# QuackenbushLab/phoenix

Measured on AMD Instinct MI355X. Metric: ODE-RHS evals/sec (genes x trajectories), higher is better.
Workload: dtype f32; 1 GPU; C4 breast_cancer ~11k-gene pseudotime, 256 trajectory intervals/GPU, dopri5 + adjoint; genes=11165, hidden=40, trajectories_per_gpu=256, method=dopri5, parallelism=trajectory-sharded x1, grouped gradient all-reduce, status_readback=deferred

## Files before the change

### phoenix_amd/csrc/phx_adj3.hip

```cpp
#include <hip/hip_runtime.h>

#include <algorithm>
#include <cstdint>
#include <cstdlib>
#include <cstring>

#include "phx_solver.hpp"
#include "phx_host.hpp"

using namespace phxh;

#include "phx_mfma_common.inc"
#include "phx_mfma_v3common.inc"
#include "phx_mfma_adj3.inc"

namespace {

int adj3_mode()
{
    if (force_v0()) return -1;
    const char *e = getenv("PHX_ADJ");
    if (!e) return 0;
    if (strcmp(e, "v3") == 0) return 1;
    if (strcmp(e, "v1") == 0 || strcmp(e, "v2") == 0) return -1;
    return 0;
}

bool plan_adj3(int N, int H, int B, int T, int control, int method, D1 *out)
{
    const int cus = num_cus();
    const int mode = adj3_mode();
    if (cus <= 0 || mode < 0 || method != PHX_DOPRI5 || H > 48) return false;
    const int HT = 3;
    const size_t blkbytes = (size_t)blk_floats_ch(HT, H) * 4;
    const int nblk = (N + 31) / 32, ntt = (B + 15) / 16;
    long long best_cost = -1;
    D1 best{};
    for (int NW = 4; NW >= 1; NW >>= 1)
        for (int TPW = 1; TPW <= 4; TPW <<= 1) {
            const int slots = NW * TPW, TG = (ntt + slots - 1) / slots;
            const int ntg = TG == 1 ? std::min(slots, ntt) : slots, Bt = 16 * ntg;
            const bool helpers = ntg < slots;
            if (control == PHX_CTRL_SHARED && TG != 1) continue;
            const size_t cb = ((ctl3_bytes(Bt, ntg) + 15) & ~(size_t)15) +
                              (v3_split_parts(TG, NW, TPW, ntg) > 1 ? v3_comb_bytes(NW, 4 * HT) : 0);
            if (cb + blkbytes > LDS_BUDGET) continue;
            const int NBmax = (int)std::min<size_t>((LDS_BUDGET - cb) / blkbytes, 8);
            const char *enb = getenv("PHX_V3_NB");
            for (int NB = enb ? std::max(1, atoi(enb)) : 1; NB <= NBmax; ++NB) {
                const int G = (nblk + NB - 1) / NB;
                if ((long long)TG * G > cus) continue;
                const long long cost = (long long)TPW * NB * 1000 + Bt / 4 - (helpers && TPW == 1 ? 50 : 0);
                if (best_cost < 0 || cost < best_cost) {
                    best_cost = cost;
                    best.N = N; best.H = H; best.B = B; best.T = T; best.HT = HT; best.NB = NB; best.NW = NW;
                    best.TPW = TPW; best.G = G; best.TG = TG; best.nblk = nblk; best.ntg = ntg; best.Bt = Bt;
                    best.nvec = NVEC_ADJ3; best.BN = (long long)B * N; best.HC = 1; best.Hc = H;
                    best.Bcall = 0; best.cntN = (long long)B * N;
                }
                break;
            }
        }
    if (best_cost < 0) return false;
    if (mode == 0 && best.G <= 32) return false;
    *out = best;
    return true;
}

size_t pp_adj3(const D1 &d) { return align_up((size_t)d.nblk * (4 * d.HT * 2 * 256) + d.N + 2 * d.H, 64); }


Regions make_layout3(const D1 &d, bool grads)
{
    Regions L{};
    Take take;
    const size_t R = (size_t)d.ntg * 4 * d.HT * 4 + d.ntg;
    L.cnt = take(4096);
    L.part = take((size_t)d.TG * d.G * R * 64 * 8);
    L.zbuf = take((size_t)d.TG * R * 64 * 8);
    L.xbytes = take.off - L.part;
    L.part1 = take((size_t)d.TG * d.G * R * 64 * 8);
    L.zbuf1 = take((size_t)d.TG * R * 64 * 8);
    L.scratch = take((size_t)d.TG * d.G * NVEC_ADJ3 * d.ntg * d.NB * 512 * 4);
    L.pp = (long long)pp_adj3(d);
    L.nparts = d.TG;
    L.dtheta = take(grads ? pp_adj3(d) * 4 * d.TG : 0);
    L.prof = take((size_t)d.TG * d.G * 16 * 8);
    L.wimg = take((size_t)d.nblk * blk_floats_ch(d.HT, d.H) * 4);
    L.hq = take(grads ? (size_t)d.TG * d.ntg * 7 * 4 * d.HT * 1024 : 0);
    L.total = take.off;
    return L;
}

size_t lds_bytes_adj3(const D1 &d)
{
    return (size_t)blk_floats_ch(d.HT, d.H) * 4 * d.NB + ((ctl3_bytes(d.Bt, d.ntg) + 15) & ~(size_t)15) +
           (v3_split_parts(d.TG, d.NW, d.TPW, d.ntg) > 1 ? v3_comb_bytes(d.NW, 4 * d.HT) : 0);
}

const void *prepare_adj3(SolveArgs &a, const phx_params *p, hipStream_t st)
{
    const D1 &d = a.d;
    if (p->wimg) a.w.wimg = (const float *)p->wimg;
    else
        hipLaunchKernelGGL(k1_pack_images, dim3(d.nblk), dim3(256), 0, st, to_net(p), (float *)a.w.wimg, d.HT, 1, p->H,
                           blk_floats_ch(d.HT, p->H));
    a.lds = lds_bytes_adj3(d);
    const char *eh = getenv("PHX_V3_HALF");
    const bool half = p->H <= 16 * (d.HT - 1) + 8 && !(eh && eh[0] == '0');
    const bool split = v3_split_parts(d.TG, d.NW, d.TPW, d.ntg) > 1;
    return split ? (half ? reinterpret_cast<const void *>(k1_solve_adj3<3, true, true>)
                         : reinterpret_cast<const void *>(k1_solve_adj3<3, false, true>))
                 : (half ? reinterpret_cast<const void *>(k1_solve_adj3<3, true, false>)
                         : reinterpret_cast<const void *>(k1_solve_adj3<3, false, false>));
}

hipError_t launch_adj3(const void *fn, const SolveArgs &a, hipStream_t st)
{
    const int flags = a.grads | (a.w.prof_level == 2 ? 2 : 0) | (a.w.prof_level == 3 ? 4 : 0);
    return launch_persistent(fn, dim3(a.d.TG * a.d.G), dim3(64 * a.d.NW), a.lds, st, a.net, a.d, a.w, a.cfg, a.t, a.y_saved,
                             a.grad_y, a.adj_y0, a.status, a.nfe, a.nsteps, flags, a.PP);
}

bool reduce_adj3(const SolveArgs &a, int npart, const phx_grads *g, int overwrite, hipStream_t st)
{
    const D1 &d = a.d;
    const long long total = (long long)d.nblk * (4 * d.HT * 2 * 64) + d.N + 2 * d.H;
    hipLaunchKernelGGL((k3_reduce_grads<3>), dim3((unsigned int)((total + 255) / 256)), dim3(256), 0, st, a.w.dtheta, npart,
                       a.PP, d.N, d.H, d.nblk, g->Ws, g->Wp, g->WaT, g->g, g->bs, g->bp, overwrite, g->Wa);
    return hipGetLastError() == hipSuccess;
}

}

namespace phxh {
const Backend &adj3_backend()
{
    static const Backend b = {3, true, false, true, plan_adj3, make_layout3, plan6_ht, prepare_adj3, launch_adj3, reduce_adj3};
    return b;
}
}
```

### phoenix_amd/csrc/phx_engine.hip

```cpp
#include <hip/hip_runtime.h>

#include <algorithm>
#include <atomic>
#include <cstdint>
#include <cstdio>
#include <cstring>
#include <cstdlib>

#include "phx_solver.hpp"
#include "phx_host.hpp"

using namespace phxh;

namespace {


struct Dims {
    int N, H, B, T;
    int NC;
    int items;
    int GB;
    int BG;
    int Bc;
    long long BN;
// ... 861 lines not shown
                     : reinterpret_cast<const void *>(k1_solve_adj<8, 256, false>);
}

hipError_t launch_v1_fwd(const void *fn, const SolveArgs &a, hipStream_t st)
{
    return launch_plain(fn, dim3(a.d.TG * a.d.G), dim3(64 * a.d.NW), a.lds, st, a.net, a.d, a.w, a.cfg, a.y0, a.t, a.sol,
                        a.status, a.nfe, a.nsteps);
}

hipError_t launch_v1_adj(const void *fn, const SolveArgs &a, hipStream_t st)
{
    return launch_plain(fn, dim3(a.d.TG * a.d.G), dim3(64 * a.d.NW), a.lds, st, a.net, a.d, a.w, a.cfg, a.t, a.y_saved,
                        a.grad_y, a.adj_y0, a.status, a.nfe, a.nsteps, a.grads, a.PP);
}

bool reduce_v1(const SolveArgs &a, int npart, const phx_grads *g, int overwrite, hipStream_t st)
{
    return launch_reduce_grads(a.w.dtheta, npart, a.PP, a.d.N, a.d.H, g, overwrite, st);
}

const Backend &v1_fwd_backend()
{
    static const Backend b = {1, false, false, false,
                                    plan_v1_fwd, layout_v1_fwd, plan6_ht, prepare_v1_fwd, launch_v1_fwd, nullptr, true};
    return b;
}
const Backend &v1_adj_backend()
{
    static const Backend b = {1, false, false, false,
                                    plan_v1_adj, layout_v1_adj, plan6_ht, prepare_v1_adj, launch_v1_adj, reduce_v1, true};
    return b;
}

const Backend *const *backends(int op)
{
    static const Backend *const fwd[] = {&fwd3_backend(), &fwd3c_backend(), &v1_fwd_backend(), nullptr};
    static const Backend *const adj[] = {&adj3_backend(), &adj3c_backend(), &adj2_backend(), &v1_adj_backend(), nullptr};
    static const Backend *const none[] = {nullptr};
    return op == PHX_OP_ODEINT ? fwd : op == PHX_OP_ADJOINT ? adj : none;
}

int pick_chunk(const Backend &be, int N, int H, int B, int T, int control, int method)
{
    D1 d;
    if (be.plan(N, H, B, T, control, method, &d)) return B;
    if (control != PHX_CTRL_PER_TRAJECTORY) return 0;
    for (int bc = 4096; bc >= 16; bc >>= 1)
        if (bc < B && be.plan(N, H, bc, T, control, method, &d)) return bc;
    return 0;
}

struct Pick {
    const Backend *be;
    int chunk;
};

Pick first_backend(int op, int N, int H, int B, int T, int control, int method, bool whole = false, bool stepped = false)
{
    for (const Backend *const *b = backends(op); *b; ++b) {
        D1 d;
        if (stepped && !(*b)->substeps) continue;
        const int chunk = !whole ? pick_chunk(**b, N, H, B, T, control, method)
                                 : (*b)->plan(N, H, B, T, control, method, &d) ? B : 0;
        if (chunk > 0) return {*b, chunk};
    }
    return {nullptr, 0};
}

SolveCfg solve_cfg(const phx_solve_opts *o)
{
    SolveCfg cfg;
    cfg.method = o->method; cfg.control = o->control; cfg.t_per_sample = o->t_per_sample; cfg.t_is_f32 = o->t_is_f32;
    cfg.rtol = (float)o->rtol; cfg.atol = (float)o->atol;
    cfg.max_steps = o->max_num_steps > 0 ? o->max_num_steps : 2147483647LL;
    cfg.step = 0.0;
    return cfg;
}

struct SolveCall {
    const phx_params *p;
    const phx_solve_opts *o;
    int B, T;
    const double *t;
    const float *y0, *y_saved, *grad_y;
    float *sol, *adj_y0;
    int *status, *nfe, *nsteps;
    const phx_grads *grads;
    void *workspace;
    size_t workspace_bytes;
    hipStream_t st;
    double step = 0.0;
    int control = -1;
    float *ckpt = nullptr;
    int Bcall = 0;
};

struct EventPair {
    hipStream_t st;
    bool open = false;
    void begin() { ev_begin(st); open = true; }
    void end()
    {
        if (open) ev_end(st);
        open = false;
    }
    ~EventPair() { end(); }
};

template <typename Plan>
int run_solve(const Backend &be, int chunk, Plan plan, const SolveCall &c)
{
    const phx_params *p = c.p;
    const phx_solve_opts *o = c.o;
    SolveArgs a{};
    a.net = to_net(p);
    a.cfg = solve_cfg(o);
    a.cfg.step = c.step;
    if (c.control >= 0) a.cfg.control = c.control;
    a.grads = c.grads ? 1 : 0;
    const char *pe = getenv("PHX_PROF");
    const int plevel = pe ? atoi(pe) : 0;
    const bool prof = be.prof_levels ? plevel >= 1 : (pe && pe[0] == '1');
    EventPair ev{c.st};
    for (int b0 = 0; b0 < c.B; b0 += chunk) {
        D1 &d = a.d;
        if (!plan(std::min(chunk, c.B - b0), &d)) return PHX_ERR_BAD_ARG;
        d.BN = (long long)c.B * p->N;
        const long long r0 = (long long)b0 * p->N;
        auto rows = [&](auto *q) { return q ? q + r0 : q; };
        a.t = !o->t_per_sample ? c.t
              : reinterpret_cast<const double *>(reinterpret_cast<const char *>(c.t) +
                                                 (size_t)(c.Bcall > 0 ? b0 / c.Bcall : b0) * c.T * (o->t_is_f32 == 2 ? 4 : 8));
        a.y0 = rows(c.y0); a.sol = rows(c.sol);
        a.y_saved = rows(c.y_saved); a.grad_y = rows(c.grad_y); a.adj_y0 = rows(c.adj_y0);
        a.status = c.status + b0; a.nfe = c.nfe + b0; a.nsteps = c.nsteps + b0;
        const Regions L = be.layout(d, c.grads != nullptr);
        if (c.workspace_bytes < L.total) return PHX_ERR_WORKSPACE;
        char *base = (char *)c.workspace;
        W1 &w = a.w;
        w.cnt = (unsigned long long *)(base + L.cnt);
        w.abort_flag = (unsigned int *)(base + L.cnt + 2048);
        w.part = (unsigned long long *)(base + L.part);
        w.zbuf = (unsigned long long *)(base + L.zbuf);
        w.part1 = (unsigned long long *)(base + L.part1);
        w.zbuf1 = (unsigned long long *)(base + L.zbuf1);
        w.scratch = (float *)(base + L.scratch);
        w.dtheta = (float *)(base + L.dtheta);
        w.prof = prof ? (unsigned long long *)(base + L.prof) : nullptr;
        w.prof_level = plevel;
        w.wimg = (const float *)(base + L.wimg);
        w.hq = (float *)(base + L.hq);
        a.PP = L.pp;
        a.ckpt = c.ckpt;
        const bool fill = !(be.cleans_idle_set && o->ws_keep && chunk >= c.B);
        if (fill && hipMemsetAsync(w.cnt, 0, L.part - L.cnt + L.xbytes, c.st) != hipSuccess) return PHX_ERR_LAUNCH;
        if (c.grads && (be.zero_dtheta_always || c.T < 2) &&
            hipMemsetAsync(w.dtheta, 0, sizeof(float) * (size_t)L.pp * L.nparts, c.st) != hipSuccess)
            return PHX_ERR_LAUNCH;
        const void *fn = be.prepare(a, p, c.st);
        if (!fn) return PHX_ERR_BAD_ARG;
        if (!set_lds_fn(fn, a.lds) || !fits_resident(fn, 64 * d.NW, a.lds, d.TG * d.G)) return PHX_ERR_LAUNCH;
        if (b0 == 0) ev.begin();
        const hipError_t lerr = be.launch(fn, a, c.st);
        if (b0 + chunk >= c.B) ev.end();
        if (lerr != hipSuccess || hipGetLastError() != hipSuccess) return PHX_ERR_LAUNCH;
        if (c.grads && !be.reduce(a, L.nparts, c.grads, (c.grads->overwrite && b0 == 0) ? 1 : 0, c.st))
            return PHX_ERR_LAUNCH;
    }
    return PHX_OK;
}

int run_solve(const Pick &k, const SolveCall &c)
{
    const Backend &be = *k.be;
    const int control = c.control >= 0 ? c.control : c.o->control;
    return run_solve(be, k.chunk, [&](int bc, D1 *d) { return be.plan(c.p->N, c.p->H, bc, c.T, control, c.o->method, d); },
                     c);
}


struct PlanEval {
    D1 d;
    int npass;
    size_t lds;
};

bool plan_eval(int N, int H, int B, int nbc_cap, PlanEval *out)
{
    const int cus = num_cus();
    if (cus <= 0 || H > 128 || force_v0()) return false;
    const int HT = H <= 48 ? 3 : 8;
    const size_t blkbytes = (size_t)blk_floats(HT, H) * 4;
    const size_t extra = 16 * 64 * 4;
    if (blkbytes + extra > LDS_BUDGET) return false;
    int NB = (int)std::min<size_t>((LDS_BUDGET - extra) / blkbytes, (size_t)nbc_cap);
    const int nblk = (N + 31) / 32, ntt = (B + 15) / 16;
    NB = std::min(NB, nblk);
    int G = (nblk + NB - 1) / NB;
    while (G > cus && NB < nbc_cap) { NB++; G = (nblk + NB - 1) / NB; }
    if (G > cus || (size_t)NB * blkbytes + extra > LDS_BUDGET) return false;
    const int NW = 4;
    int TG = std::max(1, cus / G);
    TG = std::min(TG, (ntt + NW - 1) / NW);
    D1 &d = out->d;
    d = D1{};
    d.N = N; d.H = H; d.B = B; d.T = 0; d.HT = HT; d.NB = NB; d.NW = NW; d.TPW = 1; d.G = G; d.TG = TG;
    d.nblk = nblk; d.ntg = NW; d.Bt = 16 * NW; d.nvec = 0; d.BN = (long long)B * N;
    d.HC = 1; d.Hc = H;
    out->npass = (ntt + TG * NW - 1) / (TG * NW);
    out->lds = (size_t)NB * blkbytes + extra;
    return true;
}

struct LayoutE {
    size_t total, cnt, part, zbuf, dtheta, xbytes;
};

LayoutE make_layout_eval(const PlanEval &pe, bool aug)
{
    const D1 &d = pe.d;
    LayoutE L;
    size_t off = 0;
    auto take = [&](size_t bytes) { size_t o = off; off = align_up(off + bytes, 256); return o; };
    const size_t R = (size_t)d.NW * (aug ? 4 : 2) * d.HT * 4;
    L.cnt = take(4096);
    L.part = take((size_t)d.TG * d.G * R * 64 * 8);
    L.zbuf = take((size_t)(aug ? pe.npass : 1) * d.TG * R * 64 * 8);
    L.xbytes = off - L.part;
    const size_t PP = align_up((size_t)4 * d.H * d.N + d.N + 2 * d.H, 4);
    L.dtheta = take(aug ? PP * 4 * d.TG * d.NW : 0);
    L.total = off;
    return L;
}

constexpr int EVAL_NBC_HT3_MAX = 4, EVAL_NBC_HT8 = 1;
int eval_nbc_ht3()
{
    int n = 2;
    if (const char *e = getenv("PHX_EVAL_NBC")) n = atoi(e);
    return std::min(EVAL_NBC_HT3_MAX, std::max(2, n));
}

inline int batch_fwd_min_rows(bool have_images)
{
    if (const char *e = getenv("PHX_BATCH_MIN_ROWS")) return std::max(1, atoi(e));
    return have_images ? 1 : 1024;
}
struct PlanBatch {
    D1 d;
    size_t ldsA;
    int ntiles, chunk_tiles, chunk_tiles2, KS, pgW, pgG4, slabs;
    long long Kp;
    size_t part, hdt, dtheta, total;
    size_t zl, losspart, total_fwd;
    size_t zl4, dgpart, total_vjp;
};

bool plan_batch(int N, int H, int B, PlanBatch *out)
{
    const int cus = num_cus();
    if (cus <= 0 || force_v0()) return false;
    if (const char *e = getenv("PHX_PGRAD")) if (strcmp(e, "v1") == 0) return false;
    const int HC = (H + 127) / 128, Hc = (H + HC - 1) / HC;
    const int HT = solve_ht(HC, Hc);
    const size_t blkbytes = (size_t)blk_floats_ch(HT, Hc) * 4;
    if (blkbytes > LDS_BUDGET) return false;
    const int nblk = (N + 31) / 32;
    const int NB = (int)std::min<size_t>(std::min<size_t>(LDS_BUDGET / blkbytes, 6), (size_t)nblk);
    D1 &d = out->d;
    d = D1{};
    d.N = N; d.H = H; d.B = B; d.HT = HT; d.NB = NB; d.NW = 4; d.TPW = 1; d.nblk = nblk;
    d.G = (nblk + NB - 1) / NB;
    d.TG = std::max(1, cus / d.G);
    d.HC = HC; d.Hc = Hc; d.BN = (long long)B * N;
    out->ldsA = (size_t)NB * blkbytes;
    out->ntiles = (B + 15) / 16;
    out->Kp = (long long)out->ntiles * 16;
    const size_t per_tile = (size_t)16 * HT * d.G * 64 * 4;
    auto even_chunks = [&](size_t cmax) {
        const size_t nch = ((size_t)out->ntiles + cmax - 1) / cmax;
        return (int)(((size_t)out->ntiles + nch - 1) / nch);
    };
    size_t chunk_min = 64;
    if (const char *e = getenv("PHX_BATCH_CHUNK_MIN")) chunk_min = (size_t)std::max(1, atoi(e));
    out->chunk_tiles = even_chunks(std::max<size_t>(chunk_min, ((size_t)128 << 20) / per_tile));
    out->chunk_tiles2 = even_chunks(std::max<size_t>(chunk_min, ((size_t)256 << 20) / per_tile));
    const size_t part_bytes = std::max(per_tile * out->chunk_tiles, per_tile / 2 * out->chunk_tiles2);
    out->pgG4 = 4;
    if (const char *e = getenv("PHX_PGRAD_G4")) out->pgG4 = (atoi(e) == 8 && HT == 3) ? 8 : 4;
    out->slabs = (N + 16 * out->pgG4 - 1) / (16 * out->pgG4);
    {
        int per_cu = out->pgG4 == 8 ? 2 : 4;
        if (const char *e = getenv("PHX_PGRAD_WGS")) per_cu = std::max(1, std::min(8, atoi(e)));
        const long long U = (long long)out->slabs * out->ntiles;
        const long long W = std::max<long long>(1, std::min<long long>((long long)per_cu * cus, std::max<long long>(out->slabs, U / 8)));
        const long long per = std::max<long long>(1, U / W);
        out->pgW = (int)W;
        out->KS = (int)std::min<long long>(out->ntiles, (out->ntiles + per - 1) / per + 1);
    }
    size_t off = 0;
    auto take = [&](size_t bytes) { size_t o = off; off = align_up(off + bytes, 256); return o; };
    const size_t PP = align_up((size_t)4 * H * N + N + 2 * H, 4);
    out->part = take(part_bytes);
    out->hdt = take((size_t)4 * 16 * HT * out->Kp * 4);
    out->dtheta = take(PP * 4 * out->KS);
    out->total = off;
    out->zl4 = take((size_t)out->chunk_tiles * 4 * HT * 4 * 64 * 4);
    out->dgpart = take((size_t)d.TG * 4 * N * 4);
    out->total_vjp = off;
    off = align_up(part_bytes, 256);
    out->zl = take((size_t)out->chunk_tiles2 * 2 * HT * 4 * 64 * 4);
    out->losspart = take((size_t)d.TG * d.G * 16 * sizeof(double));
    out->total_fwd = off;
    return true;
}


template <int HT>
inline int batch_threads(bool expansion = false)
// ... 744 lines not shown
```

### phoenix_amd/csrc/phx_host.hpp

```cpp
#pragma once
#include <hip/hip_runtime.h>

#include <cstdlib>
#include <cstring>
#include <map>
#include <mutex>
#include <tuple>
#include <utility>
#include <vector>

#include "phx_solver.hpp"

namespace phxh {

inline std::mutex g_mu;
inline std::map<int, int> g_cus;
inline int num_cus()
{
    int dev = 0;
    if (hipGetDevice(&dev) != hipSuccess) return 0;
    std::lock_guard<std::mutex> lk(g_mu);
    auto it = g_cus.find(dev);
    if (it != g_cus.end()) return it->second;
    int n = 0;
    if (hipDeviceGetAttribute(&n, hipDeviceAttributeMultiprocessorCount, dev) != hipSuccess) return 0;
    g_cus[dev] = n;
    return n;
}

inline std::map<std::pair<int, const void *>, size_t> g_lds_granted;
inline bool set_lds_fn(const void *fn, size_t bytes)
{
    int dev = 0;
    if (hipGetDevice(&dev) != hipSuccess) return false;
    std::lock_guard<std::mutex> lk(g_mu);
    auto key = std::make_pair(dev, fn);
    auto it = g_lds_granted.find(key);
    if (it != g_lds_granted.end() && it->second >= bytes) return true;
    if (hipFuncSetAttribute(fn, hipFuncAttributeMaxDynamicSharedMemorySize, (int)bytes) != hipSuccess) return false;
    g_lds_granted[key] = bytes;
    return true;
}
template <typename K>
inline bool set_lds(K kernel, size_t bytes) { return set_lds_fn(reinterpret_cast<const void *>(kernel), bytes); }

inline std::map<std::tuple<int, const void *, int, size_t>, int> g_occ;
inline bool fits_resident(const void *fn, int threads, size_t lds, int grid)
{
    int dev = 0;
    if (hipGetDevice(&dev) != hipSuccess) return false;
    int per_cu = -1;
    {
        std::lock_guard<std::mutex> lk(g_mu);
        auto it = g_occ.find(std::make_tuple(dev, fn, threads, lds));
        if (it != g_occ.end()) per_cu = it->second;
    }
    if (per_cu < 0) {
        int n = 0;
        if (hipOccupancyMaxActiveBlocksPerMultiprocessor(&n, fn, threads, lds) != hipSuccess) return false;
        per_cu = n;
        std::lock_guard<std::mutex> lk(g_mu);
        g_occ[std::make_tuple(dev, fn, threads, lds)] = per_cu;
    }
    return (long long)per_cu * num_cus() >= grid;
}

template <typename K>
inline bool set_lds_resident(K kernel, size_t bytes, int threads, int grid)
{
    const void *fn = reinterpret_cast<const void *>(kernel);
    return set_lds_fn(fn, bytes) && fits_resident(fn, threads, bytes, grid);
}

inline bool use_coop()
{
    const char *e = getenv("PHX_COOP");
    return e && e[0] == '1';
}
template <typename... Args>
inline hipError_t launch_persistent(const void *fn, dim3 grid, dim3 block, size_t lds, hipStream_t st, Args... args)
{
    void *argv[] = {(void *)&args...};
    if (use_coop()) return hipLaunchCooperativeKernel(fn, grid, block, argv, (unsigned int)lds, st);
    return hipLaunchKernel(fn, grid, block, argv, lds, st);
}
template <typename... Args>
inline hipError_t launch_plain(const void *fn, dim3 grid, dim3 block, size_t lds, hipStream_t st, Args... args)
{
    void *argv[] = {(void *)&args...};
    return hipLaunchKernel(fn, grid, block, argv, lds, st);
}

inline thread_local hipEvent_t g_ev_start = nullptr, g_ev_stop = nullptr;
inline std::mutex g_evq_mu;
inline std::vector<std::pair<hipEvent_t, hipEvent_t>> g_evq;
inline void ev_begin(hipStream_t st)
{
    if (!g_ev_start) {
        std::lock_guard<std::mutex> lk(g_evq_mu);
        if (!g_evq.empty()) {
            g_ev_start = g_evq.front().first;
            g_ev_stop = g_evq.front().second;
            g_evq.erase(g_evq.begin());
        }
    }
    if (g_ev_start) (void)hipEventRecord(g_ev_start, st);
}
inline void ev_end(hipStream_t st)
{
    if (g_ev_stop) (void)hipEventRecord(g_ev_stop, st);
    g_ev_start = nullptr;
    g_ev_stop = nullptr;
}

inline Net to_net(const phx_params *p) { return Net{p->Ws, p->bs, p->Wp, p->bp, p->WaT, p->g, p->N, p->H}; }

constexpr size_t LDS_BUDGET = 163840 - 1024;

inline bool force_v0()
{
    const char *e = getenv("PHX_ENGINE");
    return e && strcmp(e, "v0") == 0;
}

}

namespace phxh {

struct Regions {
    size_t total, cnt, part, zbuf, part1, zbuf1, scratch, dtheta, prof, wimg, hq;
    size_t xbytes;
    long long pp;
    int nparts;
};

struct SolveArgs {
    Net net;
    D1 d;
    W1 w;
    SolveCfg cfg;
    size_t lds;
    const double *t;
    const float *y0, *y_saved, *grad_y;
    float *sol, *adj_y0;
    int *status, *nfe, *nsteps;
    int grads;
    long long PP;
    float *ckpt;
};

struct Backend {
    int id;
    bool cleans_idle_set;
    bool zero_dtheta_always;
    bool prof_levels;
    bool (*plan)(int N, int H, int B, int T, int control, int method, D1 *out);
    Regions (*layout)(const D1 &d, bool grads);
    int (*plan6)(const D1 &d);
    const void *(*prepare)(SolveArgs &a, const phx_params *p, hipStream_t st);
    hipError_t (*launch)(const void *fn, const SolveArgs &a, hipStream_t st);
    bool (*reduce)(const SolveArgs &a, int npart, const phx_grads *g, int overwrite, hipStream_t st);
    bool substeps = false;
};

struct Take {
    size_t off = 0;
    size_t operator()(size_t bytes)
    {
        const size_t o = off;
        off = align_up(off + bytes, 256);
        return o;
    }
};

inline int plan6_ht(const D1 &d) { return d.HT; }
inline int plan6_chunked(const D1 &d) { return d.HC * 10 + d.res + 2 * d.hb + (d.split > 1 ? 4 : 0); }

const Backend &fwd3_backend();
const Backend &fwd3c_backend();
const Backend &adj2_backend();
const Backend &adj3_backend();
const Backend &adj3c_backend();
bool plan_fwd3_calls(int cus, int N, int H, int Bcall, int calls, int T, D1 *out);
bool plan_fwd3c_calls(int cus, int N, int H, int Bcall, int calls, int T, D1 *out);
const Backend &bp_backend();
int bp_chunk(int cus, int N, int H, int B, int T);
bool bp_plan(int cus, int N, int H, int B, int T, D1 *out);
size_t bp_base_bytes(int cus, int N, int H, int B, int T);

}
```

### phoenix_amd/csrc/phx_mfma_adj3.inc

```
namespace {

enum { C_Y0 = 0, C_A0 = 1, C_KY = 2, C_KA = 9 };
constexpr int NVEC_ADJ3 = 16;

__host__ __device__ inline size_t ctl3_bytes(int Bt, int ntg)
{
    return ctl_bytes(Bt) + (size_t)Bt * 8 + (size_t)Bt * 8 * 4 + (size_t)ntg * 8 + 64 + 8192 ;
}


template <int HT>
__global__ __launch_bounds__(256) void k3_reduce_grads(const float *__restrict__ dtheta, int npart, long long PP, int N, int H,
                                                       int nblk, float *gWs, float *gWp, float *gWaT, float *gg, float *gbs,
                                                       float *gbp, int overwrite, float *gWa)
{
    constexpr int NA = 4 * HT * 2;
    const long long nq = (long long)nblk * NA * 64, og = nq * 4;
    const long long tid = (long long)blockIdx.x * blockDim.x + threadIdx.x;
    if (tid < nq) {
        const int lane = (int)(tid & 63), a = (int)((tid >> 6) % NA), gb = (int)(tid / (NA * 64));
        const int li = lane & 15, lq = lane >> 4, s2 = a & 1, f = (a >> 1) % HT, m = (a >> 1) / HT;
        float4 sacc = make_float4(0.f, 0.f, 0.f, 0.f);
        int g = 0;
        for (; g + 8 <= npart; g += 8) {
            float4 v[8];
#pragma unroll
            for (int k = 0; k < 8; ++k) v[k] = reinterpret_cast<const float4 *>(dtheta + (long long)(g + k) * PP)[tid];
#pragma unroll
            for (int k = 0; k < 8; ++k) { sacc.x += v[k].x; sacc.y += v[k].y; sacc.z += v[k].z; sacc.w += v[k].w; }
        }
        for (; g + 4 <= npart; g += 4) {
            float4 v[4];
#pragma unroll
            for (int k = 0; k < 4; ++k) v[k] = reinterpret_cast<const float4 *>(dtheta + (long long)(g + k) * PP)[tid];
#pragma unroll
            for (int k = 0; k < 4; ++k) { sacc.x += v[k].x; sacc.y += v[k].y; sacc.z += v[k].z; sacc.w += v[k].w; }
        }
        for (; g < npart; ++g) {
            const float4 v = reinterpret_cast<const float4 *>(dtheta + (long long)g * PP)[tid];
            sacc.x += v.x; sacc.y += v.y; sacc.z += v.z; sacc.w += v.w;
        }
        const int gene = gb * 32 + gmapC(li, s2);
        float *dst = (m == 0) ? gWs : (m == 1 ? gWp : (m == 2 ? gWaT : gWaT + (long long)H * N));
        const float o[4] = {sacc.x, sacc.y, sacc.z, sacc.w};
        if (gWa && m >= 2) {
            if (gene < N) {
                float *q = gWa + (long long)gene * 2 * H + (m - 2) * H + 16 * f;
#pragma unroll
                for (int r = 0; r < 4; ++r) {
                    const int rr = rho16(lq, r);
                    if (16 * f + rr < H) q[rr] = overwrite ? o[r] : q[rr] + o[r];
                }
            }
        } else if (gene < N) {
#pragma unroll
            for (int r = 0; r < 4; ++r) {
                const int row = 16 * f + rho16(lq, r);
                if (row < H) {
                    float *q = dst + (long long)row * N + gene;
                    *q = overwrite ? o[r] : *q + o[r];
                }
            }
        }
    } else {
        const long long e = tid - nq;
        if (e < N + 2 * H) {
            float sacc = 0.f;
            for (int g = 0; g < npart; ++g) sacc += dtheta[(long long)g * PP + og + e];
            float *q = (e < N) ? gg + e : (e < N + H ? gbs + (e - N) : gbp + (e - N - H));
            *q = overwrite ? sacc : *q + sacc;
        }
    }
}

template <int HT, bool HALF, bool SPLIT>
__global__ __launch_bounds__(256) void k1_solve_adj3(Net net, D1 d, W1 w, SolveCfg cfg, const double *__restrict__ t,
                                                     const float *__restrict__ y_saved,
                                                     const float *__restrict__ grad_y, float *adj_y0, int *status,
                                                     int *nfe_out, int *nsteps_out, int want_grads_flags, long long PP)
{
    const int want_grads = want_grads_flags & 1;
    const bool prof_sweep = (want_grads_flags & 2) != 0, prof_quad = (want_grads_flags & 4) != 0;
    extern __shared__ __attribute__((aligned(16))) float lds[];
    const int tid = threadIdx.x, lane = tid & 63, li = lane & 15, lq = lane >> 4;
    const int wv = __builtin_amdgcn_readfirstlane(tid >> 6);
    const int grp = blockIdx.x / d.G, gt = blockIdx.x % d.G;
    const int blk0 = gt * d.NB;
    const int nbl = min(d.NB, d.nblk - blk0);
    const int N = d.N, H = d.H, B = d.B, T = d.T, Bt = d.Bt, ntg = d.ntg, G = d.G;
    const int BLKF = blk_floats_ch(HT, H);
    const int RGOFF = BLKF - 32;
    const bool shared = cfg.control == PHX_CTRL_SHARED;
    constexpr int F4 = 4 * HT, F2 = 2 * HT;
    const int nparts = SPLIT ? v3_split_parts(d.TG, d.NW, d.TPW, ntg) : 1;
    const int wtile = SPLIT ? wv % ntg : wv * d.TPW;
    const int part = SPLIT ? wv / ntg : 0;
    const int nbp = SPLIT ? (nbl + nparts - 1) / nparts : nbl;
    const int b_lo = SPLIT ? min(nbl, part * nbp) : 0, b_hi = SPLIT ? min(nbl, b_lo + nbp) : nbl;
    auto pair_live = [](int k) -> bool { return !(HALF && (k >> 1) % HT == HT - 1 && (k & 1)); };
    float *ctlbase = lds + (long long)d.NB * BLKF;
    Ctl c = carve_ctl(ctlbase, Bt);
    double *xfin = reinterpret_cast<double *>(reinterpret_cast<char *>(ctlbase) + ctl_bytes(Bt));
    float *wq = reinterpret_cast<float *>(xfin + Bt);
    int *kbs = reinterpret_cast<int *>(wq + Bt * 8);
    int *rotf = kbs + ntg;
    float *wred3 = reinterpret_cast<float *>((reinterpret_cast<size_t>(rotf + ntg) + 63) & ~(size_t)63);
    float4 *comb = reinterpret_cast<float4 *>(reinterpret_cast<char *>(ctlbase) + ((ctl3_bytes(Bt, ntg) + 15) & ~(size_t)15));
    const int RH = ntg * F4 * 4;
    const int R = RH + ntg;
    unsigned long long *xpart, *xzbuf;
    unsigned int *xabort;
    const XSet xs = xset_begin(w, grp, gt, G, R, xpart, xzbuf, xabort);
    Xchg x{xpart, xzbuf, 0, xabort, 0u, G, gt, R, false};
    const __amdgpu_buffer_rsrc_t prs = make_rsrc(x.part, (unsigned int)((size_t)G * R * 512));
    const __amdgpu_buffer_rsrc_t zrs = make_rsrc(x.zbuf, (unsigned int)((size_t)R * 512));
    const int lane16x = lane * 16;
    auto st_pair = [&](__amdgpu_buffer_rsrc_t rs, int byte_off, float v0, float v1, unsigned int tag) {
        const i32x4 u = {__float_as_int(v0), (int)tag, __float_as_int(v1), (int)tag};
        store128<16>(u, rs, lane16x, byte_off);
    };
    auto ld_pair = [&](__amdgpu_buffer_rsrc_t rs, int byte_off) -> i32x4 {
        return __builtin_amdgcn_raw_buffer_load_b128(rs, lane16x, byte_off, (int)0x80000010);
    };
    SegTimer tm;
    tm.start(w.prof != nullptr, c.tacc);
    const unsigned long long clk0 = tm.on ? (unsigned long long)clock64() : 0ull;

    constexpr int NBX = 8;
    float xinit[NBX][8], ainit[NBX][8];
    {
        const int ttl = wtile, b = grp * Bt + ttl * 16 + li;
        const long long ro = (long long)(T - 1) * d.BN + (long long)b * N;
#pragma unroll
        for (int bl = 0; bl < NBX; ++bl)
            if (bl >= b_lo && bl < b_hi && ttl < ntg) {
                const int g0 = (blk0 + bl) * 32 + gmap(lq, 0);
                row_load8(y_saved, ro, g0, N, b < B, 0.5f, xinit[bl]);
                row_load8(grad_y, ro, g0, N, b < B, 0.f, ainit[bl]);
            }
    }
    stage_images_flat(w.wimg, lds, blk0, nbl, BLKF);

    const int offR = rho16(li >> 2, li & 3) * LROW + gmap(lq, 0);
    int offC[2];
    offC[0] = rho16(lq, 0) * LROW + gmapC(li, 0);
    offC[1] = rho16(lq, 0) * LROW + gmapC(li, 1);
    const int tiles_wg = ntg * d.NB;
    float *wgbase = w.scratch + (long long)blockIdx.x * d.nvec * tiles_wg * 512;
    const int lane8 = lane * 8;
    auto tptr = [&](int v, int ttl, int bl) -> float * {
        return wgbase + ((long long)v * tiles_wg + (ttl * d.NB + bl)) * 512 + lane8;
    };
    const __amdgpu_buffer_rsrc_t trs = make_rsrc(wgbase, (unsigned int)(d.nvec * tiles_wg * 2048));
    auto toff = [&](int v, int ttl, int bl) -> int { return ((v * tiles_wg) + (ttl * d.NB + bl)) * 2048; };
    auto ring = [&](int kb, int j) -> int { const int v = kb + j; return v >= 7 ? v - 7 : v; };
    auto zrow = [&](int ttl, int f4, int r) -> u64 * {
        return x.zbuf + ((long long)(ttl * F4 + f4) * 4 + r) * 64;
    };
    const __amdgpu_buffer_rsrc_t hrs = make_rsrc(w.hq + (long long)grp * ntg * 7 * (F4 * 256),
                                                 (unsigned int)(ntg * 7 * F4 * 1024));
    auto hoff = [&](int ttl, int slot, int f) -> int { return ((ttl * 7 + slot) * F4 + f) * 1024; };
    float *dth = w.dtheta + (long long)grp * PP;
    const long long og = (long long)d.nblk * (F4 * 2 * 256), obs = og + N, obp = obs + H;

    for (int lb = tid; lb < Bt; lb += blockDim.x) {
        const int b = grp * Bt + lb;
        const bool vb = b < B;
        const TimeRow tb = trowT(t, T, cfg, shared ? 0 : (vb ? b : 0));
        float sg = 1.0f;
        int st = PHX_OK;
        if (T >= 2) {
            sg = (tb[1] < tb[0]) ? -1.0f : 1.0f;
            for (int i = 0; i + 1 < T; ++i)
                if (!((double)sg * tb[i + 1] > (double)sg * tb[i])) st = PHX_ERR_BAD_ARG;
        }
        c.sgn[lb] = sg; c.st[lb] = vb ? st : PHX_OK; c.nsteps[lb] = 0; c.nfe[lb] = 0;
        c.done[lb] = (!vb || st != PHX_OK) ? 1 : 0;
        c.accept[lb] = 0; c.fin[lb] = 0; c.out_lo[lb] = 0;
        c.dtf[lb] = 0.f; c.h0f[lb] = 0.f; c.dtp[lb] = 0.f; c.d1[lb] = 0.f; c.dt[lb] = 0.0;
        xfin[lb] = 1.0;
        for (int j = 0; j < 8; ++j) wq[lb * 8 + j] = 0.f;
    }
    for (int i = tid; i < ntg; i += blockDim.x) { kbs[i] = 0; rotf[i] = 0; }
    {
        const int ttl = wtile;
#pragma unroll
        for (int bl = 0; bl < NBX; ++bl)
            if (bl >= b_lo && bl < b_hi && ttl < ntg) {
                store8(tptr(C_Y0, ttl, bl), xinit[bl]);
                store8(tptr(C_A0, ttl, bl), ainit[bl]);
            }
    }
    for (int s = 1; s < d.TPW; ++s) {
        const int ttl = wtile + s;
        if (ttl >= ntg) continue;
        const int b = grp * Bt + ttl * 16 + li;
        for (int bl = 0; bl < nbl; ++bl) {
            float xv[8], av[8];
            const int g0 = (blk0 + bl) * 32 + gmap(lq, 0);
            const long long ro = (long long)(T - 1) * d.BN + (long long)b * N;
            row_load8(y_saved, ro, g0, N, b < B, 0.5f, xv);
            row_load8(grad_y, ro, g0, N, b < B, 0.f, av);
            store8(tptr(C_Y0, ttl, bl), xv);
            store8(tptr(C_A0, ttl, bl), av);
        }
    }
    __syncthreads();
    tm.mark(6);

    auto count_active = [&]() -> int {
        __syncthreads();
        const unsigned long long mine = __ballot(tid < Bt && !c.done[tid]);
        if (lane == 0) c.misc[4 + wv] = __popcll(mine);
        __syncthreads();
        int n = 0;
        for (int k = 0; k < d.NW; ++k) n += c.misc[4 + k];
        return n;
    };

    auto reduce_rows = [&](auto zdst, int row0, int nrows, auto comp, auto post) {
        if (G <= 16) {
            for (int u = gt + wv * G; u < nrows; u += G * d.NW) {
                const int row = row0 + u;
                const int crow = comp(u);
                const u64 *rows[16], *crows[16];
#pragma unroll
                for (int k = 0; k < 16; ++k) {
                    rows[k] = x.part + ((long long)min(k, G - 1) * R + row) * 64;
                    crows[k] = x.part + ((long long)min(k, G - 1) * R + max(crow, 0)) * 64;
                }
                float v[16];
                wait_rows<16>(x, rows, G, lane, v);
// ... 776 lines not shown
            c.rk_t0[lb] = -sg * tb[iv];
            c.rk_t1[lb] = -sg * tb[iv];
            c.accept[lb] = 0; c.fin[lb] = 0;
            c.out_lo[lb] = 0;
        }
        __syncthreads();
        {
            const unsigned int tH = ++x.tag;
            sweep(I3<0>{}, I3<0>{}, I3<1>{}, I3<0>{}, 0, 0u, tH, 0u);
            reduce_hidden();
            const unsigned int tN = ++x.tag;
            sweep(I3<0>{}, I3<1>{}, I3<0>{}, I3<1>{}, 0, tH, 0u, tN);
            norms(nv);
        }
        if (tid < Bt && !c.done[tid]) {
            c.h0f[tid] = init_h0(nv[0], nv[1]);
            c.d1[tid] = nv[1];
        }
        __syncthreads();
        {
            const unsigned int tH = ++x.tag;
            sweep(I3<1>{}, I3<0>{}, I3<1>{}, I3<0>{}, 1, 0u, tH, 0u);
            reduce_hidden();
            const unsigned int tN = ++x.tag;
            sweep(I3<1>{}, I3<1>{}, I3<0>{}, I3<2>{}, 1, tH, 0u, tN);
            norms(nv);
        }
        if (tid < Bt && !c.done[tid]) {
            const float h0 = c.h0f[tid];
            const float d2 = nv[0] / h0;
            const double dt = init_dt_ni(h0, c.d1[tid], d2);
            c.dt[tid] = dt; c.dtf[tid] = (float)dt; c.nfe[tid] += 2;
            const double t0 = c.rk_t1[tid];
            if (!(t0 + dt > t0)) { c.st[tid] = PHX_ERR_DT_UNDERFLOW; c.done[tid] = 1; }
        }
        int active = count_active();
        bool first_step = true;
        while (active > 0 && !x.aborted) {
            unsigned int tH = ++x.tag;
            sweep(I3<1>{}, I3<0>{}, I3<1>{}, I3<0>{}, 2, 0u, tH, 0u);
            reduce_hidden();
            {
                unsigned int tP = tH;
                tH = ++x.tag; sweep(I3<1>{}, I3<1>{}, I3<1>{}, I3<0>{}, 2, tP, tH, 0u, first_step ? 0 : 1); reduce_hidden(); tP = tH;
                first_step = false;
                tH = ++x.tag; sweep(I3<2>{}, I3<1>{}, I3<1>{}, I3<0>{}, 2, tP, tH, 0u); reduce_hidden(); tP = tH;
                tH = ++x.tag; sweep(I3<3>{}, I3<1>{}, I3<1>{}, I3<0>{}, 2, tP, tH, 0u); reduce_hidden(); tP = tH;
                tH = ++x.tag; sweep(I3<4>{}, I3<1>{}, I3<1>{}, I3<0>{}, 2, tP, tH, 0u); reduce_hidden(); tP = tH;
                tH = ++x.tag; sweep(I3<5>{}, I3<1>{}, I3<1>{}, I3<0>{}, 2, tP, tH, 0u); reduce_hidden(); tP = tH;
                const unsigned int tN = ++x.tag;
                sweep(I3<6>{}, I3<1>{}, I3<0>{}, I3<3>{}, 2, tP, 0u, tN);
            }
            norms(nv);
            if (tid < Bt && !c.done[tid]) {
                const int lb = tid;
                const int b = grp * Bt + lb;
                const TimeRow tb = trowT(t, T, cfg, shared ? 0 : b);
                const double sg = (double)c.sgn[lb];
                const double u_end = -sg * tb[iv - 1];
                const float ratio = nv[0];
                const int acc = (ratio <= 1.0f) ? 1 : 0;
                const double t0 = c.rk_t1[lb], dt = c.dt[lb];
                const double t1 = t0 + dt;
                c.rk_t0[lb] = t0;
                c.rk_t1[lb] = acc ? t1 : t0;
                c.accept[lb] = acc;
                c.nsteps[lb] += 1;
                const int ns = c.out_lo[lb] + 1;
                c.out_lo[lb] = ns;
                c.nfe[lb] += 6;
                const float dtf = c.dtf[lb];
                c.dtp[lb] = dtf;
                int fin = 0;
                double xx = 1.0;
                if (acc && u_end <= t1) { fin = 1; xx = (u_end - t0) / (t1 - t0); }
                xfin[lb] = xx;
                for (int j = 0; j < 8; ++j) {
                    float wj = 0.f;
                    if (acc && j < 7) {
                        double W;
                        if (!fin) W = DP_CSOL64[j];
                        else {
                            const double x2 = xx * xx, x3 = x2 * xx, x4 = x3 * xx;
                            const double d1 = (j == 0) ? 1.0 : 0.0, d7 = (j == 6) ? 1.0 : 0.0;
                            const double cj = DP_CSOL64[j], mj = DP_CMID64[j];
                            W = xx * d1 + x2 * (d7 - 4.0 * d1 - 5.0 * cj + 16.0 * mj) +
                                x3 * (5.0 * d1 - 3.0 * d7 + 14.0 * cj - 32.0 * mj) +
                                x4 * (2.0 * d7 - 2.0 * d1 - 8.0 * cj + 16.0 * mj);
                        }
                        wj = (float)(sg * (double)dtf * W);
                    }
                    wq[lb * 8 + j] = wj;
                }
                const double dtn = optimal_step_size_ni(dt, ratio);
                c.dt[lb] = dtn; c.dtf[lb] = (float)dtn;
                int dn = fin;
                if (!dn) {
                    const double tn = c.rk_t1[lb];
                    if ((long long)ns >= cfg.max_steps) { c.st[lb] = PHX_ERR_MAX_STEPS; dn = 2; }
                    else if (!(tn + dtn > tn)) { c.st[lb] = PHX_ERR_DT_UNDERFLOW; dn = 2; }
                }
                c.fin[lb] = dn;
            }
            __syncthreads();
            if (tid < ntg) {
                int ok = 1, cont = 0;
                for (int k = 0; k < 16; ++k) {
                    const int lb = tid * 16 + k;
                    const bool out = c.done[lb] || c.fin[lb] != 0;
                    const bool go = !c.done[lb] && c.accept[lb] && c.fin[lb] == 0;
                    if (!out && !go) ok = 0;
                    cont += go ? 1 : 0;
                }
                rotf[tid] = (ok && cont > 0) ? 1 : 0;
            }
            __syncthreads();
            tm.mark(9);
            quad_accept(iv);
            __syncthreads();
            if (tid < ntg && rotf[tid]) kbs[tid] = ring(kbs[tid], 6);
            if (tid < Bt && !c.done[tid] && c.fin[tid]) {
                c.done[tid] = 1;
                for (int j = 0; j < 8; ++j) wq[tid * 8 + j] = 0.f;
            }
            active = count_active();
        }
    }

    __syncthreads();
    for (int s = 0; s < d.TPW; ++s) {
        const int ttl = wtile + s;
        if (ttl >= ntg) continue;
        const int b = grp * Bt + ttl * 16 + li;
        for (int bl = b_lo; bl < b_hi; ++bl) {
            float a0[8];
            load8(tptr(C_A0, ttl, bl), a0);
            row_store8(adj_y0, (long long)b * N, (blk0 + bl) * 32 + gmap(lq, 0), N, b < B, a0);
        }
    }
    if (want_grads && gfirst) {
        for (int hb = wv; hb < 2 * nbl; hb += d.NW) {
            const int bl = hb >> 1, s2 = hb & 1;
            float4 *pn = reinterpret_cast<float4 *>(dth) + (long long)(blk0 + bl) * (F4 * 2 * 64) + lane;
            for (int mf = 0; mf < F4; ++mf) pn[(mf * 2 + s2) * 64] = make_float4(0.f, 0.f, 0.f, 0.f);
            if (li == 0)
                for (int j = 0; j < 4; ++j) {
                    const int gene = (blk0 + bl) * 32 + gmap(lq, 4 * s2 + j);
                    if (gene < N) dth[og + gene] = 0.f;
                }
        }
        if (gt == 0 && wv == 0)
            for (int h = lane; h < H; h += 64) { dth[obs + h] = 0.f; dth[obp + h] = 0.f; }
    }
    tm.mark(0);
    if (tm.on) {
        for (int i = 0; i < 16; ++i) w.prof[(long long)blockIdx.x * 16 + i] = tm.acc[i];
        w.prof[(long long)blockIdx.x * 16 + 7] = (unsigned long long)clock64() - clk0;
    }
    if (gt == 0)
        for (int lb = tid; lb < Bt; lb += blockDim.x) {
            const int b = grp * Bt + lb;
            if (b < B) {
                status[b] = x.aborted ? (int)PHX_ERR_SYNC_TIMEOUT : c.st[lb];
                nfe_out[b] = c.nfe[lb];
                nsteps_out[b] = c.nsteps[lb];
            }
        }
    xset_end(xs, grp, gt, G);
}

}
```

Baseline: 57.45 billion gene*trajectory RHS evals/s.

## Fuse adjoint gradient reduction into the persistent solve kernel tail

Adds an in-kernel epilogue to the adj3 solver. Each workgroup publishes a done flag, waits on flags from the workgroups that share its gene tile, then sums the per-trajectory-group dtheta partials for that tile straight into the gradient outputs. The separate k3_reduce_grads launch is skipped when the whole batch fits in one chunk, which removes a kernel launch and a pass over the partials. In exchange it adds a spin-wait barrier with a timeout and abort path, a flag buffer in the workspace, and reads the Grad3 struct from the kernarg segment via an offset into a mirrored args struct.

Measured after the change: 56.07 billion gene*trajectory RHS evals/s. 2.4% lower.

```diff
diff --git a/phoenix_amd/csrc/phx_adj3.hip b/phoenix_amd/csrc/phx_adj3.hip
--- a/phoenix_amd/csrc/phx_adj3.hip
+++ b/phoenix_amd/csrc/phx_adj3.hip
@@ -70,6 +70,19 @@
 size_t pp_adj3(const D1 &d) { return align_up((size_t)d.nblk * (4 * d.HT * 2 * 256) + d.N + 2 * d.H, 64); }
 
 
+size_t done3_bytes(const D1 &d) { return (size_t)2 * d.TG * d.G * sizeof(unsigned int); }
+unsigned int *done3_ptr(const SolveArgs &a)
+{
+    const size_t R = (size_t)a.d.ntg * 4 * a.d.HT * 4 + a.d.ntg;
+    return reinterpret_cast<unsigned int *>(reinterpret_cast<char *>(a.w.zbuf) + align_up((size_t)a.d.TG * R * 64 * 8, 256));
+}
+
+bool reduce_in_launch_adj3(const D1 &)
+{
+    const char *e = getenv("PHX_ADJ3_REDUCE");
+    return !(e && strcmp(e, "kernel") == 0);
+}
+
 Regions make_layout3(const D1 &d, bool grads)
 {
     Regions L{};
@@ -78,6 +91,7 @@
     L.cnt = take(4096);
     L.part = take((size_t)d.TG * d.G * R * 64 * 8);
     L.zbuf = take((size_t)d.TG * R * 64 * 8);
+    take(done3_bytes(d));
     L.xbytes = take.off - L.part;
     L.part1 = take((size_t)d.TG * d.G * R * 64 * 8);
     L.zbuf1 = take((size_t)d.TG * R * 64 * 8);
@@ -117,9 +131,13 @@
 
 hipError_t launch_adj3(const void *fn, const SolveArgs &a, hipStream_t st)
 {
-    const int flags = a.grads | (a.w.prof_level == 2 ? 2 : 0) | (a.w.prof_level == 3 ? 4 : 0);
+    const phx_grads *g = a.grads ? a.gout : nullptr;
+    const int flags = a.grads | (a.w.prof_level == 2 ? 2 : 0) | (a.w.prof_level == 3 ? 4 : 0) | (g ? 8 : 0);
+    Grad3 go{};
+    if (g) go = Grad3{g->Ws, g->Wp, g->WaT, g->g, g->bs, g->bp, g->Wa, nullptr, a.gover};
+    go.done = done3_ptr(a);
     return launch_persistent(fn, dim3(a.d.TG * a.d.G), dim3(64 * a.d.NW), a.lds, st, a.net, a.d, a.w, a.cfg, a.t, a.y_saved,
-                             a.grad_y, a.adj_y0, a.status, a.nfe, a.nsteps, flags, a.PP);
+                             a.grad_y, a.adj_y0, a.status, a.nfe, a.nsteps, flags, a.PP, go);
 }
 
 bool reduce_adj3(const SolveArgs &a, int npart, const phx_grads *g, int overwrite, hipStream_t st)
@@ -136,7 +154,8 @@
 namespace phxh {
 const Backend &adj3_backend()
 {
-    static const Backend b = {3, true, false, true, plan_adj3, make_layout3, plan6_ht, prepare_adj3, launch_adj3, reduce_adj3};
+    static const Backend b = {3, true, false, true, plan_adj3, make_layout3, plan6_ht, prepare_adj3, launch_adj3, reduce_adj3,
+                              false, reduce_in_launch_adj3};
     return b;
 }
 }
diff --git a/phoenix_amd/csrc/phx_engine.hip b/phoenix_amd/csrc/phx_engine.hip
--- a/phoenix_amd/csrc/phx_engine.hip
+++ b/phoenix_amd/csrc/phx_engine.hip
@@ -1037,6 +1037,9 @@
         w.hq = (float *)(base + L.hq);
         a.PP = L.pp;
         a.ckpt = c.ckpt;
+        const bool fused = c.grads && chunk >= c.B && be.reduce_in_launch && be.reduce_in_launch(d);
+        a.gout = fused ? c.grads : nullptr;
+        a.gover = c.grads && c.grads->overwrite ? 1 : 0;
         const bool fill = !(be.cleans_idle_set && o->ws_keep && chunk >= c.B);
         if (fill && hipMemsetAsync(w.cnt, 0, L.part - L.cnt + L.xbytes, c.st) != hipSuccess) return PHX_ERR_LAUNCH;
         if (c.grads && (be.zero_dtheta_always || c.T < 2) &&
@@ -1049,7 +1052,7 @@
         const hipError_t lerr = be.launch(fn, a, c.st);
         if (b0 + chunk >= c.B) ev.end();
         if (lerr != hipSuccess || hipGetLastError() != hipSuccess) return PHX_ERR_LAUNCH;
-        if (c.grads && !be.reduce(a, L.nparts, c.grads, (c.grads->overwrite && b0 == 0) ? 1 : 0, c.st))
+        if (c.grads && !fused && !be.reduce(a, L.nparts, c.grads, (c.grads->overwrite && b0 == 0) ? 1 : 0, c.st))
             return PHX_ERR_LAUNCH;
     }
     return PHX_OK;
diff --git a/phoenix_amd/csrc/phx_host.hpp b/phoenix_amd/csrc/phx_host.hpp
--- a/phoenix_amd/csrc/phx_host.hpp
+++ b/phoenix_amd/csrc/phx_host.hpp
@@ -147,6 +147,8 @@
     int grads;
     long long PP;
     float *ckpt;
+    const phx_grads *gout;
+    int gover;
 };
 
 struct Backend {
@@ -161,6 +163,7 @@
     hipError_t (*launch)(const void *fn, const SolveArgs &a, hipStream_t st);
     bool (*reduce)(const SolveArgs &a, int npart, const phx_grads *g, int overwrite, hipStream_t st);
     bool substeps = false;
+    bool (*reduce_in_launch)(const D1 &d) = nullptr;
 };
 
 struct Take {
diff --git a/phoenix_amd/csrc/phx_mfma_adj3.inc b/phoenix_amd/csrc/phx_mfma_adj3.inc
--- a/phoenix_amd/csrc/phx_mfma_adj3.inc
+++ b/phoenix_amd/csrc/phx_mfma_adj3.inc
@@ -73,11 +73,111 @@
     }
 }
 
+struct Grad3 {
+    float *Ws, *Wp, *WaT, *g, *bs, *bp, *Wa;
+    unsigned int *done;
+    int overwrite;
+};
+
+template <int HT>
+__device__ __noinline__ void adj3_reduce_tile(const float *dtheta, int npart, long long PP, int N, int H, int nblk, int blk0,
+                                              int nbl, int grp, int bias, Grad3 go)
+{
+    constexpr int NA = 4 * HT * 2;
+    constexpr int U = 5;
+    const int tid = threadIdx.x, lane = tid & 63, li = lane & 15, lq = lane >> 4;
+    const int wv = __builtin_amdgcn_readfirstlane(tid >> 6), nw = (int)blockDim.x >> 6;
+    const int nslot = nbl * NA, stride = npart * nw;
+    const long long og = (long long)nblk * NA * 256;
+    for (int s0 = grp + npart * wv; s0 < nslot; s0 += U * stride) {
+        float4 sacc[U];
+        long long idx[U];
+#pragma unroll
+        for (int k = 0; k < U; ++k) {
+            sacc[k] = make_float4(0.f, 0.f, 0.f, 0.f);
+            idx[k] = ((long long)blk0 * NA + min(s0 + k * stride, nslot - 1)) * 64 + lane;
+        }
+        int g = 0;
+        for (; g + 4 <= npart; g += 4) {
+            float4 v[U][4];
+#pragma unroll
+            for (int k = 0; k < U; ++k)
+#pragma unroll
+                for (int j = 0; j < 4; ++j) v[k][j] = reinterpret_cast<const float4 *>(dtheta + (long long)(g + j) * PP)[idx[k]];
+#pragma unroll
+            for (int k = 0; k < U; ++k)
+#pragma unroll
+                for (int j = 0; j < 4; ++j) { sacc[k].x += v[k][j].x; sacc[k].y += v[k][j].y; sacc[k].z += v[k][j].z; sacc[k].w += v[k][j].w; }
+        }
+        for (; g < npart; ++g) {
+            float4 v[U];
+#pragma unroll
+            for (int k = 0; k < U; ++k) v[k] = reinterpret_cast<const float4 *>(dtheta + (long long)g * PP)[idx[k]];
+#pragma unroll
+            for (int k = 0; k < U; ++k) { sacc[k].x += v[k].x; sacc[k].y += v[k].y; sacc[k].z += v[k].z; sacc[k].w += v[k].w; }
+        }
+#pragma unroll
+        for (int k = 0; k < U; ++k) {
+            const int sl = s0 + k * stride;
+            if (sl >= nslot) break;
+            const int a = sl % NA, gb = blk0 + sl / NA;
+            const int s2 = a & 1, f = (a >> 1) % HT, m = (a >> 1) / HT;
+            const int gene = gb * 32 + gmapC(li, s2);
+            if (gene >= N) continue;
+            const float o[4] = {sacc[k].x, sacc[k].y, sacc[k].z, sacc[k].w};
+            if (go.Wa && m >= 2) {
+                float *q = go.Wa + (long long)gene * 2 * H + (m - 2) * H + 16 * f;
+#pragma unroll
+                for (int r = 0; r < 4; ++r) {
+                    const int rr = rho16(lq, r);
+                    if (16 * f + rr < H) q[rr] = go.overwrite ? o[r] : q[rr] + o[r];
+                }
+            } else {
+                float *dst = (m == 0) ? go.Ws : (m == 1 ? go.Wp : (m == 2 ? go.WaT : go.WaT + (long long)H * N));
+#pragma unroll
+                for (int r = 0; r < 4; ++r) {
+                    const int row = 16 * f + rho16(lq, r);
+                    if (row < H) {
+                        float *q = dst + (long long)row * N + gene;
+                        *q = go.overwrite ? o[r] : *q + o[r];
+                    }
+                }
+            }
+        }
+    }
+    for (int i = grp + npart * tid; i < nbl * 32; i += npart * (int)blockDim.x) {
+        const int gene = blk0 * 32 + i;
+        if (gene >= N) break;
+        float sacc = 0.f;
+        for (int g = 0; g < npart; ++g) sacc += dtheta[(long long)g * PP + og + gene];
+        go.g[gene] = go.overwrite ? sacc : go.g[gene] + sacc;
+    }
+    if (bias)
+        for (int e = tid; e < 2 * H; e += (int)blockDim.x) {
+            float sacc = 0.f;
+            for (int g = 0; g < npart; ++g) sacc += dtheta[(long long)g * PP + og + N + e];
+            float *q = e < H ? go.bs + e : go.bp + (e - H);
+            *q = go.overwrite ? sacc : *q + sacc;
+        }
+}
+
+struct Adj3Args {
+    Net net; D1 d; W1 w; SolveCfg cfg;
+    const double *t;
+    const float *y_saved, *grad_y;
+    float *adj_y0;
+    int *status, *nfe_out, *nsteps_out;
+    int want_grads_flags;
+    long long PP;
+    Grad3 go;
+};
+
 template <int HT, bool HALF, bool SPLIT>
 __global__ __launch_bounds__(256) void k1_solve_adj3(Net net, D1 d, W1 w, SolveCfg cfg, const double *__restrict__ t,
                                                      const float *__restrict__ y_saved,
                                                      const float *__restrict__ grad_y, float *adj_y0, int *status,
-                                                     int *nfe_out, int *nsteps_out, int want_grads_flags, long long PP)
+                                                     int *nfe_out, int *nsteps_out, int want_grads_flags, long long PP,
+                                                     Grad3 )
 {
     const int want_grads = want_grads_flags & 1;
     const bool prof_sweep = (want_grads_flags & 2) != 0, prof_quad = (want_grads_flags & 4) != 0;
@@ -1160,6 +1260,51 @@
         if (gt == 0 && wv == 0)
             for (int h = lane; h < H; h += 64) { dth[obs + h] = 0.f; dth[obp + h] = 0.f; }
     }
+    {
+        typedef const __attribute__((address_space(4))) Grad3 *KGrad3;
+        typedef const __attribute__((address_space(4))) char *KBytes;
+        const KGrad3 kg = (KGrad3)((KBytes)__builtin_amdgcn_kernarg_segment_ptr() + offsetof(Adj3Args, go));
+        const Grad3 go{kg->Ws, kg->Wp, kg->WaT, kg->g, kg->bs, kg->bp, kg->Wa, kg->done, kg->overwrite};
+        const unsigned int nwg = gridDim.x;
+        if (tid == 0) go.done[(1u - xs.s) * nwg + blockIdx.x] = 0u;
+        if (want_grads_flags & 8) {
+            unsigned int *flags = go.done + xs.s * nwg;
+            asm volatile("s_waitcnt vmcnt(0)" ::: "memory");
+            __syncthreads();
+            if (tid == 0) {
+                __builtin_amdgcn_fence(__ATOMIC_RELEASE, "agent");
+                asm volatile("s_waitcnt vmcnt(0)" ::: "memory");
+                __hip_atomic_store(&flags[blockIdx.x], 1u, __ATOMIC_RELAXED, __HIP_MEMORY_SCOPE_AGENT);
+            }
+            if (wv == 0) {
+                unsigned int spins = 0;
+                unsigned long long t_start = 0;
+                while (!x.aborted) {
+                    bool ok = true;
+                    for (int k = lane; k < d.TG; k += 64)
+                        ok = ok && __hip_atomic_load(&flags[k * G + gt], __ATOMIC_RELAXED, __HIP_MEMORY_SCOPE_AGENT) != 0u;
+                    if (__all(ok)) break;
+                    __builtin_amdgcn_s_sleep(2);
+                    if ((++spins & 255u) == 0) {
+                        if (t_start == 0) t_start = wall_clock64();
+                        if (__hip_atomic_load(x.abort_flag, __ATOMIC_RELAXED, __HIP_MEMORY_SCOPE_AGENT) ||
+                            wall_clock64() - t_start > 500000000ull) {
+                            __hip_atomic_store(x.abort_flag, 1u, __ATOMIC_RELAXED, __HIP_MEMORY_SCOPE_AGENT);
+                            x.aborted = true;
+                        }
+                    }
+                }
+                if (!x.aborted) {
+                    __builtin_amdgcn_fence(__ATOMIC_ACQUIRE, "agent");
+                    asm volatile("s_waitcnt vmcnt(0)" ::: "memory");
+                }
+                if (lane == 0) c.misc[2] = x.aborted ? 0 : 1;
+            }
+            __syncthreads();
+            if (c.misc[2]) adj3_reduce_tile<HT>(w.dtheta, d.TG, PP, N, H, d.nblk, blk0, nbl, grp, (gt == 0 && grp == 0) ? 1 : 0, go);
+            else x.aborted = true;
+        }
+    }
     tm.mark(0);
     if (tm.on) {
         for (int i = 0; i < 16; ++i) w.prof[(long long)blockIdx.x * 16 + i] = tm.acc[i];
```
